# bridgedp/hunter_bipedal_control

Measured on NVIDIA H100. Metric: MPC+WBC control-step solves/sec (Hunter N=100), higher is better.
Workload: dtype f64

## Files before the change

hunter_bipedal_control_b200/csrc/hb_qp.cuh:

```cuda
#pragma once
#include "hb_common.cuh"

namespace hb {

constexpr int QP_MAX_N = 80;
constexpr int QP_MAX_EQ = 32;
constexpr int QP_MAX_IN = 96;
constexpr int QP_MAX_M = 160;

struct QpWorkspace {
  double *H, *Aeq, *K, *V, *S;
  double *kdi, *sdi;
  double *g, *x, *rd, *dx, *t1, *t2;
  double *beq, *y, *rp, *dy, *t3;
  double *f, *s, *z, *rs, *ds, *dz, *rc, *sgn, *wt;
  int *in_row, *in_c0, *in_c1, *in_pair, *ord, *eq_row;
  int ldn, ldv, lds;
  int me_cap, mi_cap;
};

__host__ __device__ constexpr int qp_ld(int n) { return n | 1; }

__host__ __device__ constexpr int tri_row(int i) { return i * (i + 1) / 2; }

__host__ __device__ constexpr size_t qp_workspace_doubles(int n, int me_cap = QP_MAX_EQ, int mi_cap = QP_MAX_IN, bool packed_h = false) {
  const int ldn = qp_ld(n), lde = me_cap | 1;
  size_t d = 0;
  d += packed_h ? (size_t)tri_row(n) : (size_t)n * ldn;
  d += (size_t)me_cap * ldn;
  d += (size_t)n * ldn;
  d += (size_t)n * lde;
  d += (size_t)me_cap * lde;
  d += n + me_cap;
  d += 6 * (size_t)n;
  d += 5 * (size_t)me_cap;
  d += 9 * (size_t)mi_cap;
  d += (5 * (size_t)mi_cap + me_cap + 1) / 2 + 1;
  return d;
}

__device__ inline void qp_carve(double* base, int n, QpWorkspace& w, int me_cap = QP_MAX_EQ, int mi_cap = QP_MAX_IN, bool packed_h = false) {
  const int ldn = qp_ld(n), lde = me_cap | 1;
  w.ldn = ldn; w.ldv = lde; w.lds = lde; w.me_cap = me_cap; w.mi_cap = mi_cap;
  double* p = base;
  w.H = p; p += packed_h ? tri_row(n) : n * ldn;
  w.Aeq = p; p += me_cap * ldn;
  w.K = p; p += n * ldn;
  w.V = p; p += n * lde;
  w.S = p; p += me_cap * lde;
  w.kdi = p; p += n;
  w.sdi = p; p += me_cap;
  w.g = p; p += n; w.x = p; p += n; w.rd = p; p += n; w.dx = p; p += n; w.t1 = p; p += n; w.t2 = p; p += n;
  w.beq = p; p += me_cap; w.y = p; p += me_cap; w.rp = p; p += me_cap; w.dy = p; p += me_cap; w.t3 = p; p += me_cap;
  w.f = p; p += mi_cap; w.s = p; p += mi_cap; w.z = p; p += mi_cap; w.rs = p; p += mi_cap;
  w.ds = p; p += mi_cap; w.dz = p; p += mi_cap; w.rc = p; p += mi_cap; w.sgn = p; p += mi_cap; w.wt = p; p += mi_cap;
  int* ip = reinterpret_cast<int*>(p);
  w.in_row = ip; ip += mi_cap; w.in_c0 = ip; ip += mi_cap; w.in_c1 = ip; ip += mi_cap; w.in_pair = ip; ip += mi_cap; w.ord = ip; ip += mi_cap; w.eq_row = ip;
}

__device__ inline bool warp_chol_inv(double* M, int n, int ld, double* invdiag, int lane, double piv_floor = 0.0) {
  bool ok = true;
  for (int j = 0; j < n; ++j) {
    for (int i = j + lane; i < n; i += 32) {
      const double* ri = M + i * ld;
      const double* rj = M + j * ld;
      double a0 = ri[j], a1 = 0.0, a2 = 0.0, a3 = 0.0;
      int k = 0;
      for (; k + 3 < j; k += 4) {
        a0 -= ri[k] * rj[k]; a1 -= ri[k + 1] * rj[k + 1]; a2 -= ri[k + 2] * rj[k + 2]; a3 -= ri[k + 3] * rj[k + 3];
      }
      for (; k < j; ++k) a0 -= ri[k] * rj[k];
      M[i * ld + j] = (a0 + a1) + (a2 + a3);
    }
    __syncwarp();
    double d = M[j * ld + j];
    if (!(d > piv_floor)) {
      if (piv_floor > 0.0 && d == d) d = piv_floor; else { ok = false; d = 1.0; }
    }
    const double r = 1.0 / sqrt(d);
    __syncwarp();
    for (int i = j + lane; i < n; i += 32) M[i * ld + j] *= r;
    if (lane == 0) invdiag[j] = r;
    __syncwarp();
  }
  for (int c0 = 0; c0 < n; c0 += 32) {
    const int c = c0 + lane;
    const bool act = c < n;
    for (int i = c0 + 1; i < n; ++i) {
      if (act && i > c) {
        const double* Li_row = M + i * ld;
        double* col = M + c * ld;
        double a0 = Li_row[c] * invdiag[c], a1 = 0.0;
        int k = c + 1;
        for (; k + 1 < i; k += 2) { a0 += Li_row[k] * col[k]; a1 += Li_row[k + 1] * col[k + 1]; }
        if (k < i) a0 += Li_row[k] * col[k];
        col[i] = -(a0 + a1) * invdiag[i];
      }
    }
  }
  __syncwarp();
  return ok;
}

template <int LD, int W, int WMAX>
__device__ __forceinline__ void chol_window_factor(double (&a)[WMAX], double* M, int& j, int jend, int n, double* invdiag, int lane,
                                                   double piv_floor, bool& ok) {
  for (; j < jend; ++j) {
    double d = __shfl_sync(HB_FULL_MASK, a[0], j);
    if (!(d > piv_floor)) { if (piv_floor > 0.0 && d == d) d = piv_floor; else { ok = false; d = 1.0; } }
    const double r = rsqrt(d);
    const double l = a[0] * r;
    if (lane < n) M[lane * LD + j] = l;
    if (lane == j) invdiag[j] = r;
    __syncwarp();
    const double* col = M + (j + 1) * LD + j;
#pragma unroll
    for (int k = 0; k < W - 1; ++k) a[k] = fma(-l, col[k * LD], a[k + 1]);
  }
}

template <int LD, int W, int WMAX>
__device__ __forceinline__ void chol_window_inverse(double (&res)[WMAX], double* M, int& j, int jend, const double* invdiag, int lane) {
  for (; j < jend; ++j) {
    const double y = res[0] * invdiag[j];
    if (lane < j) M[lane * LD + j] = y;
    const double* col = M + (j + 1) * LD + j;
#pragma unroll
    for (int k = 0; k < W - 1; ++k) res[k] = fma(-col[k * LD], y, res[k + 1]);
  }
}

template <int LD, int WMAX>
__device__ __noinline__ bool warp_chol_inv_window(double* M, int n, double* invdiag, int lane, double piv_floor) {
  static_assert(WMAX <= 32 && WMAX % 7 == 0, "one lane per row, stages of seven columns");
  bool ok = true;
  double a[WMAX];
#pragma unroll
  for (int c = 0; c < WMAX; ++c) a[c] = (lane < n && c <= lane) ? M[lane * LD + c] : 0.0;
  __syncwarp();
  int j = 0;
  if constexpr (WMAX >= 28) chol_window_factor<LD, 28, WMAX>(a, M, j, n - 21, n, invdiag, lane, piv_floor, ok);
  if constexpr (WMAX >= 21) chol_window_factor<LD, 21, WMAX>(a, M, j, n - 14, n, invdiag, lane, piv_floor, ok);
  if constexpr (WMAX >= 14) chol_window_factor<LD, 14, WMAX>(a, M, j, n - 7, n, invdiag, lane, piv_floor, ok);
  chol_window_factor<LD, 7, WMAX>(a, M, j, n, n, invdiag, lane, piv_floor, ok);
  __syncwarp();
#pragma unroll
  for (int c = 0; c < WMAX; ++c) a[c] = (c == lane) ? 1.0 : 0.0;
  j = 0;
  if constexpr (WMAX >= 28) chol_window_inverse<LD, 28, WMAX>(a, M, j, n - 21, invdiag, lane);
  if constexpr (WMAX >= 21) chol_window_inverse<LD, 21, WMAX>(a, M, j, n - 14, invdiag, lane);
  if constexpr (WMAX >= 14) chol_window_inverse<LD, 14, WMAX>(a, M, j, n - 7, invdiag, lane);
  chol_window_inverse<LD, 7, WMAX>(a, M, j, n, invdiag, lane);
  __syncwarp();
  return ok;
}

__device__ inline bool warp_chol_inv_any(double* M, int n, int ld, double* invdiag, int lane, double piv_floor) {
  if (ld == 29 && n <= 28) return warp_chol_inv_window<29, 28>(M, n, invdiag, lane, piv_floor);
  if (ld == 7 && n <= 7) return warp_chol_inv_window<7, 7>(M, n, invdiag, lane, piv_floor);
  return warp_chol_inv(M, n, ld, invdiag, lane, piv_floor);
}

__device__ inline void warp_li_mv(const double* M, int n, int ld, const double* invdiag, const double* v, double* y, int lane) {
  for (int i = lane; i < n; i += 32) {
    double a0 = invdiag[i] * v[i], a1 = 0.0;
    int k = 0;
    for (; k + 1 < i; k += 2) { a0 += M[k * ld + i] * v[k]; a1 += M[(k + 1) * ld + i] * v[k + 1]; }
    if (k < i) a0 += M[k * ld + i] * v[k];
    y[i] = a0 + a1;
  }
  __syncwarp();
}
__device__ inline void warp_lit_mv(const double* M, int n, int ld, const double* invdiag, const double* v, double* y, int lane) {
  for (int i = lane; i < n; i += 32) {
    const double* row = M + i * ld;
    double a0 = invdiag[i] * v[i], a1 = 0.0;
    int k = i + 1;
    for (; k + 1 < n; k += 2) { a0 += row[k] * v[k]; a1 += row[k + 1] * v[k + 1]; }
    if (k < n) a0 += row[k] * v[k];
    y[i] = a0 + a1;
  }
  __syncwarp();
}

struct QpResult { int status; int iters; };

template <class Bound, class Residuals, class Factor, class Newton, class Step>
__device__ __forceinline__ QpResult qp_mehrotra_warp(int mi, int max_iter, double gs, double bs, double fsum, double* s, double* z, double* ds,
                                                     double* dz, double* rc, Bound bound, Residuals residuals, Factor factor, Newton newton,
                                                     Step step) {
  const int lane = lane_id();
  fsum = warp_sum(fsum);
  const double theta = fmax(1.0, mi > 0 ? fsum / mi : 1.0);
  for (int j = lane; j < mi; j += 32) { const double sj = fmax(theta, bound(j)); s[j] = sj; z[j] = theta / sj; }
  gs = warp_max(gs); bs = warp_max(bs);
  __syncwarp();
  auto max_step = [&]() {
    double a = 1.0;
    for (int j = lane; j < mi; j += 32) {
      if (ds[j] < 0.0) a = fmin(a, -s[j] / ds[j]);
      if (dz[j] < 0.0) a = fmin(a, -z[j] / dz[j]);
    }
    return warp_min(a);
  };
  QpResult res{1, 0};
  int it = 0;
  for (; it < max_iter; ++it) {
    double rdn = 0.0, rpn = 0.0;
    const double sz = residuals(rdn, rpn);
    rdn = warp_max(rdn); rpn = warp_max(rpn);
    const double mu = mi > 0 ? warp_sum(sz) / mi : 0.0;
    if (!(rdn == rdn) || !(rpn == rpn) || !(mu == mu) || rdn > 1e300 || rpn > 1e300) { res.status = 3; break; }
    if (rdn < 1e-10 * gs && rpn < 1e-10 * bs && mu < 1e-12) { res.status = 0; break; }
    if (!factor()) { res.status = 2; break; }
    for (int j = lane; j < mi; j += 32) rc[j] = s[j] * z[j];
    __syncwarp();
    newton();
    if (mi > 0) {
      const double a_aff = max_step();
      double ma = 0.0;
      for (int j = lane; j < mi; j += 32) ma += (s[j] + a_aff * ds[j]) * (z[j] + a_aff * dz[j]);
      ma = warp_sum(ma) / mi;
      const double r = ma / mu;
      const double sigma = r * r * r;
      for (int j = lane; j < mi; j += 32) rc[j] = s[j] * z[j] + ds[j] * dz[j] - sigma * mu;
      __syncwarp();
      newton();
    }
    const double alpha = fmin(1.0, 0.995 * max_step());
    step(alpha);
    for (int j = lane; j < mi; j += 32) { s[j] += alpha * ds[j]; z[j] += alpha * dz[j]; }
    __syncwarp();
  }
  res.iters = it;
  return res;
}

template <bool PACKED_H = false>
__device__ inline QpResult qp_solve_warp(int n, int m, const double* __restrict__ H, const double* __restrict__ g,
                                         const double* __restrict__ A, const double* __restrict__ lbA,
                                         const double* __restrict__ ubA, double rho, int max_iter, double* x_out,
                                         QpWorkspace& w) {
  const int lane = lane_id();
  const int ldn = w.ldn, ldv = w.ldv, lds = w.lds;
  int me = 0, mi = 0;
  bool infeasible = false;
  for (int r0 = 0; r0 < m; r0 += 32) {
    const int r = r0 + lane;
    int c0 = n, c1 = 0;
    double lo = 0.0, hi = 0.0;
    if (r < m) {
      const double* a = A + (size_t)r * n;
      for (int c = 0; c < n; ++c) if (a[c] != 0.0) { if (c < c0) c0 = c; c1 = c + 1; }
      lo = lbA[r]; hi = ubA[r];
    }
    const bool valid = r < m;
    const bool zero_row = valid && c1 == 0;
    const bool has_lo = valid && lo > -1e19, has_hi = valid && hi < 1e19;
    if (zero_row && ((has_lo && lo > 1e-12) || (has_hi && hi < -1e-12))) infeasible = true;
    const bool is_eq = valid && !zero_row && has_lo && has_hi && lo == hi;
    const bool up = valid && !zero_row && !is_eq && has_hi;
    const bool dn = valid && !zero_row && !is_eq && has_lo;
    const unsigned beq = __ballot_sync(HB_FULL_MASK, is_eq);
    const unsigned bup = __ballot_sync(HB_FULL_MASK, up);
    const unsigned bdn = __ballot_sync(HB_FULL_MASK, dn);
    const unsigned below = (1u << lane) - 1u;
    if (is_eq) { const int e = me + __popc(beq & below); if (e < w.me_cap) { w.eq_row[e] = r; w.beq[e] = hi; } }
    const int mi2 = mi + __popc(bup);
    const int e_up = mi + __popc(bup & below), e_dn = mi2 + __popc(bdn & below);
    if (up && e_up < w.mi_cap) { w.in_row[e_up] = r; w.in_c0[e_up] = c0; w.in_c1[e_up] = c1; w.sgn[e_up] = 1.0; w.f[e_up] = hi; w.in_pair[e_up] = (dn && e_dn < w.mi_cap) ? e_dn : -1; }
    if (dn && e_dn < w.mi_cap) { w.in_row[e_dn] = r; w.in_c0[e_dn] = c0; w.in_c1[e_dn] = c1; w.sgn[e_dn] = -1.0; w.f[e_dn] = -lo; w.in_pair[e_dn] = up ? -2 : -1; }
    me += __popc(beq);
    mi = mi2 + __popc(bdn);
  }
  infeasible = __any_sync(HB_FULL_MASK, infeasible);
  QpResult res{1, 0};
  if (infeasible) res.status = 2;
  else if (me > w.me_cap || mi > w.mi_cap || n > QP_MAX_N) res.status = 4;
  if (res.status != 1) {
    for (int i = lane; i < n; i += 32) x_out[i] = 0.0;
    return res;
  }
  __syncwarp();
  int nwide = 0, nact = 0;
  for (int pass = 0; pass < 2; ++pass) {
    for (int j0 = 0; j0 < mi; j0 += 32) {
      const int j = j0 + lane;
      const bool sel = j < mi && w.in_pair[j] != -2 && ((w.in_c1[j] - w.in_c0[j] > 8) == (pass == 0));
      const unsigned msk = __ballot_sync(HB_FULL_MASK, sel);
      if (sel) w.ord[nact + __popc(msk & ((1u << lane) - 1u))] = j;
      nact += __popc(msk);
    }
    if (pass == 0) nwide = nact;
  }
  __syncwarp();
  const bool colmask = n <= 32 && nact - nwide <= 32;
  unsigned nmask = 0u;
  if (colmask && lane < n)
    for (int q = nwide; q < nact; ++q) { const int j = w.ord[q]; if (lane >= w.in_c0[j] && lane < w.in_c1[j]) nmask |= 1u << (q - nwide); }
  auto at_mul = [&](int i, double a) {
    for (int q = 0; q < nwide; ++q) { const int j = w.ord[q]; a = fma(w.wt[j], A[(size_t)w.in_row[j] * n + i], a); }
    if (colmask) {
      for (unsigned mk = nmask; mk; mk &= mk - 1u) { const int j = w.ord[nwide + __ffs(mk) - 1]; a = fma(w.wt[j], A[(size_t)w.in_row[j] * n + i], a); }
      return a;
    }
    for (int q = nwide; q < nact; ++q) {
      const int j = w.ord[q];
      if (i >= w.in_c0[j] && i < w.in_c1[j]) a = fma(w.wt[j], A[(size_t)w.in_row[j] * n + i], a);
    }
    return a;
  };
  if (H != nullptr) for (int idx = lane; idx < n * n; idx += 32) { const int i = idx / n, c = idx - i * n; w.H[i * ldn + c] = H[idx]; }
  for (int e = 0; e < me; ++e) {
    const double* a = A + (size_t)w.eq_row[e] * n;
    for (int c = lane; c < n; c += 32) w.Aeq[e * ldn + c] = a[c];
  }
  double gs = 1.0, bs = 1.0;
  for (int i = lane; i < n; i += 32) { const double gi = g[i]; w.g[i] = gi; w.x[i] = 0.0; gs = fmax(gs, 1.0 + fabs(gi)); }
  for (int e = lane; e < me; e += 32) { w.y[e] = 0.0; bs = fmax(bs, 1.0 + fabs(w.beq[e])); }
  double fsum = 0.0;
  for (int j = lane; j < mi; j += 32) { fsum += fabs(w.f[j]); bs = fmax(bs, 1.0 + fabs(w.f[j])); }
  auto residuals = [&](double& rdn, double& rpn) {
    for (int j = lane; j < mi; j += 32) {
      const int pr = w.in_pair[j];
      double cj = w.sgn[j] * w.z[j];
      if (pr >= 0) cj += w.sgn[pr] * w.z[pr];
      w.wt[j] = cj;
    }
    __syncwarp();
    for (int i = lane; i < n; i += 32) {
      double a = w.g[i] + rho * w.x[i];
      if (PACKED_H) {
        const double* hr = w.H + tri_row(i);
        for (int c = 0; c <= i; ++c) a += hr[c] * w.x[c];
        for (int c = i + 1; c < n; ++c) a += w.H[tri_row(c) + i] * w.x[c];
      } else {
        const double* hr = w.H + i * ldn;
        for (int c = 0; c < n; ++c) a += hr[c] * w.x[c];
      }
      for (int e = 0; e < me; ++e) a += w.Aeq[e * ldn + i] * w.y[e];
      w.rd[i] = at_mul(i, a);
    }
    for (int e = lane; e < me; e += 32) {
      double a = -w.beq[e];
      for (int c = 0; c < n; ++c) a += w.Aeq[e * ldn + c] * w.x[c];
      w.rp[e] = a;
    }
    double sz = 0.0;
    for (int j = lane; j < mi; j += 32) {
      const double* a = A + (size_t)w.in_row[j] * n;
      double d = 0.0;
      for (int c = w.in_c0[j]; c < w.in_c1[j]; ++c) d += a[c] * w.x[c];
      w.rs[j] = w.sgn[j] * d + w.s[j] - w.f[j];
      sz += w.s[j] * w.z[j];
    }
    __syncwarp();
    for (int i = lane; i < n; i += 32) rdn = fmax(rdn, fabs(w.rd[i]));
    for (int e = lane; e < me; e += 32) rpn = fmax(rpn, fabs(w.rp[e]));
    for (int j = lane; j < mi; j += 32) rpn = fmax(rpn, fabs(w.rs[j]));
    return sz;
  };
  auto factor = [&]() {
    if (PACKED_H) {
      for (int idx = lane; idx < n * ldn; idx += 32) { const int i = idx / ldn, c = idx - i * ldn; if (c <= i) w.K[idx] = w.H[tri_row(i) + c] + ((i == c) ? rho : 0.0); }
    } else {
      for (int idx = lane; idx < n * ldn; idx += 32) { const int i = idx / ldn, c = idx - i * ldn; w.K[idx] = w.H[idx] + ((i == c) ? rho : 0.0); }
    }
    __syncwarp();
    for (int j = lane; j < mi; j += 32) {
      const int pr = w.in_pair[j];
      double wj = w.z[j] / w.s[j];
      if (pr >= 0) wj += w.z[pr] / w.s[pr];
      w.wt[j] = wj;
    }
    __syncwarp();
    {
      constexpr int WCH = 10;
      for (int cb = 0; cb < n; cb += 32) {
        const int c = cb + lane;
        const bool act = c < n;
        for (int q0 = 0; q0 < nwide; q0 += WCH) {
          double t[WCH]; int roff[WCH];
#pragma unroll
          for (int q = 0; q < WCH; ++q) {
            const bool on = q0 + q < nwide;
            const int j = on ? w.ord[q0 + q] : 0;
            roff[q] = on ? w.in_row[j] * n : 0;
            t[q] = (on && act) ? w.wt[j] * A[(size_t)roff[q] + c] : 0.0;
          }
          for (int i = cb; i < n; ++i) {
            double acc = 0.0;
#pragma unroll
            for (int q = 0; q < WCH; ++q) acc = fma(t[q], A[(size_t)roff[q] + i], acc);
            if (act && i >= c) w.K[i * ldn + c] += acc;
          }
        }
      }
    }
    __syncwarp();
    if (colmask) {
      for (unsigned mk = nmask; mk; mk &= mk - 1u) {
        const int j = w.ord[nwide + __ffs(mk) - 1];
        const int c1 = w.in_c1[j];
        const double wj = w.wt[j];
        const double* a = A + (size_t)w.in_row[j] * n;
        const double ac = a[lane];
        for (int i = lane; i < c1; ++i) w.K[i * ldn + lane] += (wj * a[i]) * ac;
      }
      __syncwarp();
    } else
    for (int q = nwide; q < nact; ++q) {
      const int j = w.ord[q];
      const int c0 = w.in_c0[j], c1 = w.in_c1[j];
      const double wj = w.wt[j];
      const double* a = A + (size_t)w.in_row[j] * n;
      for (int i = c0; i < c1; ++i) {
        const double ai = wj * a[i];
        for (int c = c0 + lane; c <= i; c += 32) w.K[i * ldn + c] += ai * a[c];
      }
      __syncwarp();
    }
    bool ok = warp_chol_inv_any(w.K, n, ldn, w.kdi, lane, 1e-10);
    if (me > 0) {
      for (int idx = lane; idx < n * me; idx += 32) {
        const int i = idx / me, e = idx - i * me;
        const double* ar = w.Aeq + e * ldn;
        double a0 = w.kdi[i] * ar[i], a1 = 0.0;
        int k = 0;
        for (; k + 1 < i; k += 2) { a0 += w.K[k * ldn + i] * ar[k]; a1 += w.K[(k + 1) * ldn + i] * ar[k + 1]; }
        if (k < i) a0 += w.K[k * ldn + i] * ar[k];
        w.V[i * ldv + e] = a0 + a1;
      }
      __syncwarp();
      for (int idx = lane; idx < me * me; idx += 32) {
        const int a = idx / me, b = idx - a * me;
        if (b <= a) {
          double s0 = 0.0, s1 = 0.0;
          int i = 0;
          for (; i + 1 < n; i += 2) { s0 += w.V[i * ldv + a] * w.V[i * ldv + b]; s1 += w.V[(i + 1) * ldv + a] * w.V[(i + 1) * ldv + b]; }
          if (i < n) s0 += w.V[i * ldv + a] * w.V[i * ldv + b];
          w.S[a * lds + b] = s0 + s1;
        }
      }
      __syncwarp();
      ok = warp_chol_inv_any(w.S, me, lds, w.sdi, lane, 1e-14) && ok;
    }
    return ok;
  };
  auto newton = [&]() {
    for (int j = lane; j < mi; j += 32) {
      const int pr = w.in_pair[j];
      double cj = w.sgn[j] * ((w.rc[j] - w.z[j] * w.rs[j]) / w.s[j]);
      if (pr >= 0) cj += w.sgn[pr] * ((w.rc[pr] - w.z[pr] * w.rs[pr]) / w.s[pr]);
      w.wt[j] = cj;
    }
    __syncwarp();
    for (int i = lane; i < n; i += 32) w.t2[i] = at_mul(i, -w.rd[i]);
    __syncwarp();
    warp_li_mv(w.K, n, ldn, w.kdi, w.t2, w.t1, lane);
    if (me > 0) {
      for (int e = lane; e < me; e += 32) {
        double a = w.rp[e];
        for (int i = 0; i < n; ++i) a += w.V[i * ldv + e] * w.t1[i];
        w.t3[e] = a;
      }
      __syncwarp();
      warp_li_mv(w.S, me, lds, w.sdi, w.t3, w.dy, lane);
      for (int e = lane; e < me; e += 32) w.t3[e] = w.dy[e];
      __syncwarp();
      warp_lit_mv(w.S, me, lds, w.sdi, w.t3, w.dy, lane);
      for (int i = lane; i < n; i += 32) {
        double a = w.t1[i];
        for (int e = 0; e < me; ++e) a -= w.V[i * ldv + e] * w.dy[e];
        w.t2[i] = a;
      }
      __syncwarp();
    } else {
      for (int i = lane; i < n; i += 32) w.t2[i] = w.t1[i];
      __syncwarp();
    }
    warp_lit_mv(w.K, n, ldn, w.kdi, w.t2, w.dx, lane);
    for (int j = lane; j < mi; j += 32) {
      const double* a = A + (size_t)w.in_row[j] * n;
      double d = 0.0;
      for (int c = w.in_c0[j]; c < w.in_c1[j]; ++c) d += a[c] * w.dx[c];
      const double dsj = -w.rs[j] - w.sgn[j] * d;
      w.ds[j] = dsj;
      w.dz[j] = -(w.rc[j] + w.z[j] * dsj) / w.s[j];
    }
    __syncwarp();
  };
  auto step = [&](double alpha) {
    for (int i = lane; i < n; i += 32) w.x[i] += alpha * w.dx[i];
    for (int e = lane; e < me; e += 32) w.y[e] += alpha * w.dy[e];
  };
  res = qp_mehrotra_warp(mi, max_iter, gs, bs, fsum, w.s, w.z, w.ds, w.dz, w.rc, [&](int j) { return w.f[j]; }, residuals, factor, newton, step);
  for (int i = lane; i < n; i += 32) x_out[i] = w.x[i];
  return res;
}

}

namespace {
using namespace hb;
__global__ void qp_batch_kernel(int B, int n, int m, const double* H, const double* g, const double* A, const double* lbA, const double* ubA,
                                size_t strideH, size_t strideA, size_t strideB, const int32_t* m_per, double rho, int max_iter, double* x,
                                int32_t* status, int32_t* iters) {
  extern __shared__ __align__(16) unsigned char smem_raw[];
  const int warp = threadIdx.x >> 5, wpb = blockDim.x >> 5;
  const int inst = blockIdx.x * wpb + warp;
  if (inst >= B) return;
  double* base = reinterpret_cast<double*>(smem_raw) + (size_t)warp * qp_workspace_doubles(n);
  QpWorkspace w;
  qp_carve(base, n, w);
  const int mi = m_per ? m_per[inst] : m;
  QpResult r = qp_solve_warp(n, mi, H + inst * strideH, g + (size_t)inst * n, A + inst * strideA, lbA + inst * strideB, ubA + inst * strideB,
                             rho, max_iter, x + (size_t)inst * n, w);
  if (lane_id() == 0) { if (status) status[inst] = r.status; if (iters) iters[inst] = r.iters; }
}
}
```

hunter_bipedal_control_b200/csrc/hb_wbc.cuh:

```cuda
#pragma once
#include "hb_common.cuh"
#include "hb_planner.h"
#include "hb_qp.cuh"
#include "hb_rbd.cuh"
#include "../../include/hunter_b200.h"

namespace hb {

constexpr int WBC_ROWS = 60;
constexpr double QP_INFTY = 1e20;

struct WbcShared {
  double J[12 * 16];
  double Ad[6 * 16];
  double M[16 * 16];
  double nle[16];
  double q[16], v[16], qd[16], vd[16];
  double pos_m[12], vel_m[12], dJv[12], pos_d[12], vel_d[12];
  double Adv[6], com_d[3];
  double At[18 * 16];
  double bt[18];
  double misc[32];
  double frame[36];
};

struct WbcRows {
  int nc, nsw;
  int eq;
  int md0;
  int nt;
  int ma2;
  int m;
};
__device__ inline WbcRows wbc_rows(int mode, bool stance_mode) {
  int nc = 0;
  for (int c = 0; c < 4; ++c) nc += contact_flag(mode, c);
  const int nsw = 4 - nc, eq = 16 + 3 * nsw, md0 = 2 * NJ + 5 * nc;
  return {nc, nsw, eq, md0, stance_mode ? 6 : 3 * nsw + 6, 12 + 3 * nsw, eq + md0 + 3 * nsw};
}
constexpr int WBC_MA0 = 28;

__device__ inline void rotation_error_world(const double* Rref, const double* Rmeas, double* err) {
  double E[9];
  for (int i = 0; i < 3; ++i)
    for (int j = 0; j < 3; ++j) E[3 * i + j] = Rref[3 * i] * Rmeas[3 * j] + Rref[3 * i + 1] * Rmeas[3 * j + 1] + Rref[3 * i + 2] * Rmeas[3 * j + 2];
  const double sk[3] = {E[7] - E[5], E[2] - E[6], E[3] - E[1]};
  double c = 0.5 * (E[0] + E[4] + E[8] - 1.0);
  c = fmin(1.0, fmax(-1.0, c));
  const double ang = acos(c);
  const double sn = sqrt(sk[0] * sk[0] + sk[1] * sk[1] + sk[2] * sk[2]);
  double f = 0.5;
  if (ang > 1e-8 && sn > 1e-12) f = ang / sn;
  for (int i = 0; i < 3; ++i) err[i] = f * sk[i];
}

__device__ inline void wbc_contact_frames(const hb_terrain& m, WbcShared& sh) {
  const int c = lane_id();
  if (c >= 4) return;
  double* f = sh.frame + 9 * c;
  if (!hbplan::map_frame(m, sh.pos_m[3 * c], sh.pos_m[3 * c + 1], f)) f[2] = 0.0;
}

__device__ __forceinline__ const double* wbc_frames(const InstanceView<hb_terrain>& maps, int inst, const WbcShared& sh) {
  return maps.of(inst) ? sh.frame : nullptr;
}

__device__ inline int wbc_terms_warp(const double* __restrict__ x_des, const double* __restrict__ u_des, const double* __restrict__ rbd,
                                     int mode, const bool& stance_mode, const hb_wbc_settings& ws, const InstanceView<hb_terrain>& maps, int inst,
                                     WbcShared& sh) {
  const int lane = lane_id();
  const Model& md = c_model;
  if (lane == 0) {
    rbd_to_qv(rbd, sh.q, sh.v);
    for (int i = 0; i < NQ; ++i) sh.qd[i] = x_des[6 + i];
  }
  __syncwarp();
  {
    double q[NQ], e[NQ];
    const bool meas = lane < 16;
    const int k = lane & 15;
    for (int i = 0; i < NQ; ++i) { q[i] = meas ? sh.q[i] : sh.qd[i]; e[i] = (i == k) ? 1.0 : 0.0; }
    KinOut<double> o;
    kin_pass<double>(q, e, o);
    if (meas) { for (int r = 0; r < 12; ++r) sh.J[r * 16 + k] = o.cvel[r]; }
    else { for (int r = 0; r < 6; ++r) sh.Ad[r * 16 + k] = o.h[r]; }
  }
  __syncwarp();
  if (lane == 0) {
    double Ab[36], rhs[6], vb[6];
    for (int r = 0; r < 6; ++r) {
      for (int c = 0; c < 6; ++c) Ab[6 * r + c] = sh.Ad[r * 16 + c];
      double s = md.total_mass * x_des[r];
      for (int j = 0; j < NJ; ++j) s -= sh.Ad[r * 16 + 6 + j] * u_des[12 + j];
      rhs[r] = s;
    }
    solve6_cmm(Ab, rhs, vb);
    for (int i = 0; i < 6; ++i) sh.vd[i] = vb[i];
    for (int j = 0; j < NJ; ++j) sh.vd[6 + j] = u_des[12 + j];
  }
  __syncwarp();
  if (lane < 2) {
    D1 q[NQ], v[NQ];
    for (int i = 0; i < NQ; ++i) {
      const double qi = lane == 0 ? sh.q[i] : sh.qd[i], vi = lane == 0 ? sh.v[i] : sh.vd[i];
      q[i] = D1(qi, vi); v[i] = D1(vi, 0.0);
    }
    KinOut<D1> o;
    kin_pass<D1>(q, v, o);
    if (lane == 0) { for (int r = 0; r < 12; ++r) { sh.pos_m[r] = o.cpos[r].v; sh.vel_m[r] = o.cvel[r].v; sh.dJv[r] = o.cvel[r].d; } }
    else {
      for (int r = 0; r < 12; ++r) { sh.pos_d[r] = o.cpos[r].v; sh.vel_d[r] = o.cvel[r].v; }
      for (int r = 0; r < 6; ++r) sh.Adv[r] = o.h[r].d;
      for (int r = 0; r < 3; ++r) sh.com_d[r] = o.com[r].v;
    }
  }
  if (lane < 17) {
    double q[NQ], v[NQ], a[NQ], tau[NQ];
    for (int i = 0; i < NQ; ++i) { q[i] = sh.q[i]; v[i] = lane == 16 ? sh.v[i] : 0.0; a[i] = (i == lane) ? 1.0 : 0.0; }
    rnea_pass(q, v, a, lane == 16, tau, nullptr);
    if (lane < 16) { for (int r = 0; r < NQ; ++r) sh.M[r * 16 + lane] = tau[r]; }
    else { for (int r = 0; r < NQ; ++r) sh.nle[r] = tau[r]; }
  }
  __syncwarp();
  if (const hb_terrain* m = maps.of(inst)) wbc_contact_frames(*m, sh);
  for (int idx = lane; idx < 256; idx += 32) {
    const int i = idx >> 4, j = idx & 15;
    if (j < i) { const double a = 0.5 * (sh.M[i * 16 + j] + sh.M[j * 16 + i]); sh.M[i * 16 + j] = a; }
  }
  __syncwarp();
  for (int idx = lane; idx < 256; idx += 32) { const int i = idx >> 4, j = idx & 15; if (j > i) sh.M[i * 16 + j] = sh.M[j * 16 + i]; }
  __syncwarp();
  if (lane == 0) {
    bool fl[4];
    for (int c = 0; c < 4; ++c) fl[c] = contact_flag(mode, c);
    for (int i = 0; i < 18 * 16; ++i) sh.At[i] = 0.0;
    if (stance_mode) {
      for (int i = 0; i < 6; ++i) { sh.At[i * 16 + i] = 1.0; sh.bt[i] = 0.0; }
    } else {
      double hd[6] = {0, 0, 0, 0, 0, 0};
      for (int c = 0; c < 4; ++c) {
        const double* F = u_des + 3 * c;
        const double r0 = sh.pos_d[3 * c] - sh.com_d[0], r1 = sh.pos_d[3 * c + 1] - sh.com_d[1], r2 = sh.pos_d[3 * c + 2] - sh.com_d[2];
        hd[0] += F[0]; hd[1] += F[1]; hd[2] += F[2];
        hd[3] += r1 * F[2] - r2 * F[1]; hd[4] += r2 * F[0] - r0 * F[2]; hd[5] += r0 * F[1] - r1 * F[0];
      }
      hd[2] -= md.total_mass * HB_GRAVITY;
      double Ab[36], rhs[6], qbdd[6];
      for (int r = 0; r < 6; ++r) { for (int c = 0; c < 6; ++c) Ab[6 * r + c] = sh.Ad[r * 16 + c]; rhs[r] = hd[r] - sh.Adv[r]; }
      solve6_cmm(Ab, rhs, qbdd);
      double Rd[9], axd[9], Rm[9], axm[9];
      base_frame<double>(sh.qd, Rd, axd);
      base_frame<double>(sh.q, Rm, axm);
      double baseVelW[3], baseAccW[3], wm[3], dJw_v[3];
      {
        const double* vd = sh.vd;
        double w1[3], w2[3], t1[3], t2[3];
        for (int i = 0; i < 3; ++i) { w1[i] = axd[i] * vd[3]; w2[i] = w1[i] + axd[3 + i] * vd[4]; }
        cross(w1, &axd[3], t1); cross(w2, &axd[6], t2);
        for (int i = 0; i < 3; ++i) {
          baseVelW[i] = w2[i] + axd[6 + i] * vd[5];
          baseAccW[i] = axd[i] * qbdd[3] + axd[3 + i] * qbdd[4] + axd[6 + i] * qbdd[5] + t1[i] * vd[4] + t2[i] * vd[5];
        }
      }
      {
        const double* vm = sh.v;
        double w1[3], w2[3], t1[3], t2[3];
        for (int i = 0; i < 3; ++i) { w1[i] = axm[i] * vm[3]; w2[i] = w1[i] + axm[3 + i] * vm[4]; }
        cross(w1, &axm[3], t1); cross(w2, &axm[6], t2);
        for (int i = 0; i < 3; ++i) { wm[i] = w2[i] + axm[6 + i] * vm[5]; dJw_v[i] = t1[i] * vm[4] + t2[i] * vm[5]; }
      }
      int r = 0;
      for (int c = 0; c < 4; ++c) if (!fl[c]) for (int a = 0; a < 3; ++a) {
        const double acc = ws.swing_kp * (sh.pos_d[3 * c + a] - sh.pos_m[3 * c + a]) + ws.swing_kd * (sh.vel_d[3 * c + a] - sh.vel_m[3 * c + a]);
        for (int j = 0; j < NQ; ++j) sh.At[r * 16 + j] = sh.J[(3 * c + a) * 16 + j];
        sh.bt[r] = acc - sh.dJv[3 * c + a];
        ++r;
      }
      for (int a = 0; a < 2; ++a) { sh.At[r * 16 + a] = 1.0; sh.bt[r] = qbdd[a]; ++r; }
      sh.At[r * 16 + 2] = 1.0;
      sh.bt[r] = qbdd[2] + ws.base_height_kp * (sh.qd[2] - sh.q[2]) + ws.base_height_kd * (sh.vd[2] - sh.v[2]);
      ++r;
      double err[3];
      rotation_error_world(Rd, Rm, err);
      for (int a = 0; a < 3; ++a) {
        for (int i = 0; i < 3; ++i) sh.At[r * 16 + 3 + i] = axm[3 * i + a];
        sh.bt[r] = baseAccW[a] + ws.base_angular_kp * err[a] + ws.base_angular_kd * (baseVelW[a] - wm[a]) - dJw_v[a];
        ++r;
      }
    }
  }
  __syncwarp();
  return wbc_rows(mode, stance_mode).nt;
}

__device__ inline void wbc_weight_rows(WbcShared& sh, const WbcRows& n, bool stance_mode, const hb_wbc_settings& ws) {
  const int lane = lane_id(), nsr = stance_mode ? 0 : 3 * n.nsw;
  for (int idx = lane; idx < n.nt * 16; idx += 32) sh.At[idx] *= (idx >> 4) < nsr ? ws.weight_swing_leg : ws.weight_base_accel;
  for (int r = lane; r < n.nt; r += 32) sh.bt[r] *= r < nsr ? ws.weight_swing_leg : ws.weight_base_accel;
  __syncwarp();
}

__device__ inline const hb_wbc_settings& wbc_select_settings(const hb_wbc_settings& ws, InstanceView<hb_controller_setting> cs, int inst,
                                                             hb_wbc_settings& dst) {
  if (lane_id() == 0) {
    const hb_controller_setting* c = cs.of(inst);
    if (c) dst = c->wbc;
    else dst = ws;
  }
  __syncwarp();
  return dst;
}

__device__ inline int wbc_nth_contact(int mode, bool stance, int k) {
  int c = 0;
  for (; c < 3; ++c) if (contact_flag(mode, c) == stance && k-- == 0) break;
  return c;
}

__device__ inline void wbc_task0_eq(const WbcShared& sh, int mode, const WbcRows& n, int rows, double* A, int lda, double* b) {
  const int lane = lane_id(), nsw = n.nsw;
  for (int idx = lane; idx < rows * NWBC; idx += 32) {
    const int i = idx / NWBC, j = idx - i * NWBC;
    double a = 0.0;
    if (i < 16) {
      if (j < NQ) a = sh.M[i * 16 + j];
      else if (j < NQ + 12) a = -sh.J[(j - NQ) * 16 + i];
      else a = (i >= 6 && j - NQ - 12 == i - 6) ? -1.0 : 0.0;
    } else if (i < 16 + 3 * nsw) {
      const int k = i - 16, c = wbc_nth_contact(mode, false, k / 3);
      a = (j == NQ + 3 * c + k % 3) ? 1.0 : 0.0;
    } else {
      const int k = i - 16 - 3 * nsw, c = wbc_nth_contact(mode, true, k / 3);
      a = j < NQ ? sh.J[(3 * c + k % 3) * 16 + j] : 0.0;
    }
    A[i * lda + j] = a;
  }
  for (int i = lane; i < rows; i += 32) {
    double v = 0.0;
    if (i < 16) v = -sh.nle[i];
    else if (i >= 16 + 3 * nsw) { const int k = i - 16 - 3 * nsw; v = -sh.dJv[3 * wbc_nth_contact(mode, true, k / 3) + k % 3]; }
    b[i] = v;
  }
}

__device__ inline double wbc_task0_ineq(const hb_wbc_settings& ws, int mode, int q, int& col0, int& len, double* coef, const double* frames) {
  if (q < 2 * NJ) {
    const int j = q % NJ;
    col0 = NQ + 12 + j; len = 1; coef[0] = q < NJ ? 1.0 : -1.0; coef[1] = 0.0; coef[2] = 0.0;
    return ws.torque_limits[j % 5];
  }
  const int fr = q - 2 * NJ, k = fr % 5;
  const double mu = ws.friction_coefficient;
  const int c = wbc_nth_contact(mode, true, fr / 5);
  col0 = NQ + 3 * c; len = 3;
  const double* f = frames ? frames + 9 * c : nullptr;
  if (f && f[2] != 0.0) {
    const double* t = f + (k < 3 ? 3 : 6);
    for (int a = 0; a < 3; ++a) coef[a] = k == 0 ? -f[a] : (k & 1 ? t[a] : -t[a]) - hbplan::mul_rn(mu, f[a]);
    return 0.0;
  }
  coef[0] = k == 1 ? 1.0 : (k == 2 ? -1.0 : 0.0);
  coef[1] = k == 3 ? 1.0 : (k == 4 ? -1.0 : 0.0);
  coef[2] = k == 0 ? -1.0 : -mu;
  return 0.0;
}

__device__ inline int wbc_task12_rows(int lvl, const double* At, const double* bt, const WbcRows& n, const double* u_des, double* A, int lda, double* b) {
  const int lane = lane_id(), nswr = 3 * n.nsw;
  const int ma = lvl == 1 ? 6 : n.ma2;
  for (int idx = lane; idx < ma * NWBC; idx += 32) {
    const int i = idx / NWBC, j = idx - i * NWBC;
    double a = 0.0;
    if (lvl == 1) { if (j < NQ) a = At[(nswr + i) * 16 + j]; }
    else if (i < 12) a = (j == NQ + i) ? 0.1 : 0.0;
    else if (j < NQ) a = At[(i - 12) * 16 + j];
    A[i * lda + j] = a;
  }
  for (int i = lane; i < ma; i += 32) b[i] = lvl == 1 ? bt[nswr + i] : (i < 12 ? 0.1 * u_des[i] : bt[i - 12]);
  return ma;
}

__device__ inline int wbc_reduced_build(const WbcShared& sh, const WbcRows& n, int mode, bool stance_mode, double rho, const hb_wbc_settings& ws,
                                        const double* frames, const double* __restrict__ u_des, double* Hw, double* gz, double* Az, double* lbz,
                                        double* ubz, int* stcol , int& m_out) {
  const int lane = lane_id();
  if (lane == 0) for (int j = 0, k = 0; j < 12; ++j) if (contact_flag(mode, j / 3)) stcol[k++] = j;
  const int nz = NQ + 3 * n.nc, m = 6 + NJ + 5 * n.nc, nw = n.nt;
  __syncwarp();
  for (int idx = lane; idx < m * nz; idx += 32) {
    const int r = idx / nz, c = idx - r * nz;
    double v = 0.0;
    if (r < 6 + NJ) v = (c < NQ) ? sh.M[r * 16 + c] : -sh.J[stcol[c - NQ] * 16 + r];
    else {
      const int fr = r - 6 - NJ, ci = fr / 5;
      const int cc = c - NQ - 3 * ci;
      if (cc >= 0 && cc < 3) { int c0, len; double coef[3]; wbc_task0_ineq(ws, mode, 2 * NJ + fr, c0, len, coef, frames); v = coef[cc]; }
    }
    Az[idx] = v;
  }
  for (int r = lane; r < m; r += 32) {
    int c0, len; double coef[3];
    if (r < 6) { lbz[r] = -sh.nle[r]; ubz[r] = -sh.nle[r]; }
    else if (r < 6 + NJ) { const int j = r - 6; const double lim = wbc_task0_ineq(ws, mode, j, c0, len, coef, nullptr); lbz[r] = -lim - sh.nle[6 + j]; ubz[r] = lim - sh.nle[6 + j]; }
    else { lbz[r] = -QP_INFTY; ubz[r] = wbc_task0_ineq(ws, mode, NJ + r - 6, c0, len, coef, frames); }
  }
  __syncwarp();
  const double* Tm = Az + 6 * nz;
  const double wf2 = stance_mode ? 0.0 : ws.weight_contact_force * ws.weight_contact_force;
  for (int idx = lane; idx < nz * nz; idx += 32) {
    const int i = idx / nz, j = idx - i * nz;
    if (j > i) continue;
    double s = (i == j) ? rho : 0.0;
    if (i == j && i >= NQ) s += wf2;
    if (i < NQ && j < NQ) for (int r = 0; r < nw; ++r) s += sh.At[r * 16 + i] * sh.At[r * 16 + j];
    double t = 0.0;
    for (int r = 0; r < NJ; ++r) t += Tm[r * nz + i] * Tm[r * nz + j];
    Hw[tri_row(i) + j] = s + rho * t;
  }
  for (int i = lane; i < nz; i += 32) {
    double s = 0.0;
    if (i < NQ) for (int r = 0; r < nw; ++r) s -= sh.At[r * 16 + i] * sh.bt[r];
    else s = -wf2 * u_des[stcol[i - NQ]];
    double t = 0.0;
    for (int r = 0; r < NJ; ++r) t += Tm[r * nz + i] * sh.nle[6 + r];
    gz[i] = s + rho * t;
  }
  __syncwarp();
  m_out = m;
  return nz;
}

}

namespace {
using namespace hb;
constexpr int QP_STRIDE_H = NWBC * NWBC, QP_STRIDE_A = WBC_ROWS * NWBC;

__global__ void wbc_assemble_kernel(int B, hb_wbc_settings ws, const __grid_constant__ InstanceView<hb_terrain> maps, const double* x_des,
                                    const double* u_des, const double* rbd, const int32_t* mode, const uint8_t* stance_mode, double* H, double* g,
                                    double* A, double* lbA, double* ubA, int32_t* m_out) {
  extern __shared__ __align__(16) unsigned char smem_raw[];
  const int warp = threadIdx.x >> 5, wpb = blockDim.x >> 5;
  const int inst = blockIdx.x * wpb + warp;
  if (inst >= B) return;
  WbcShared& sh = reinterpret_cast<WbcShared*>(smem_raw)[warp];
  const int md = mode[inst];
  const bool stance = stance_mode ? stance_mode[inst] != 0 : false;
  const double* ud = u_des + (size_t)inst * NU;
  wbc_terms_warp(x_des + (size_t)inst * NX, ud, rbd + (size_t)inst * 32, md, stance, ws, maps, inst, sh);
  const WbcRows n = wbc_rows(md, stance);
  wbc_weight_rows(sh, n, stance, ws);
  const int lane = lane_id();
  H += (size_t)inst * QP_STRIDE_H; g += (size_t)inst * NWBC; A += (size_t)inst * QP_STRIDE_A; lbA += (size_t)inst * WBC_ROWS; ubA += (size_t)inst * WBC_ROWS;
  const double wf2 = stance ? 0.0 : ws.weight_contact_force * ws.weight_contact_force;
  for (int idx = lane; idx < NWBC * NWBC; idx += 32) {
    const int i = idx / NWBC, j = idx - i * NWBC;
    double s = 0.0;
    if (i < NQ && j < NQ) for (int r = 0; r < n.nt; ++r) s += sh.At[r * 16 + i] * sh.At[r * 16 + j];
    if (i == j && i >= NQ && i < NQ + 12) s += wf2;
    H[idx] = s;
  }
  for (int i = lane; i < NWBC; i += 32) {
    double s = 0.0;
    if (i < NQ) for (int r = 0; r < n.nt; ++r) s += sh.At[r * 16 + i] * sh.bt[r];
    else if (i < NQ + 12) s = wf2 * ud[i - NQ];
    g[i] = -s;
  }
  for (int idx = lane; idx < n.m * NWBC; idx += 32) A[idx] = 0.0;
  __syncwarp();
  wbc_task0_eq(sh, md, n, n.eq, A, NWBC, lbA);
  for (int q = lane; q < n.md0; q += 32) {
    int c0, len; double coef[3];
    const int r = n.eq + q;
    ubA[r] = wbc_task0_ineq(ws, md, q, c0, len, coef, wbc_frames(maps, inst, sh));
    lbA[r] = -QP_INFTY;
    for (int k = 0; k < len; ++k) A[r * NWBC + c0 + k] = coef[k];
  }
  for (int r = n.eq + n.md0 + lane; r < n.m; r += 32) { lbA[r] = -QP_INFTY; ubA[r] = 0.0; }
  __syncwarp();
  for (int i = lane; i < n.eq; i += 32) ubA[i] = lbA[i];
  if (lane == 0) m_out[inst] = n.m;
}

constexpr int WZ_N = 28, WZ_ME = 6, WZ_MI = 40, WZ_ROWS = 36;
__host__ __device__ constexpr size_t wbc_fused_doubles() { return qp_workspace_doubles(WZ_N, WZ_ME, WZ_MI, true) + WZ_ROWS * WZ_N + 2 * WZ_ROWS + 3 * WZ_N + 16 + 8; }
static_assert(8 * (wbc_fused_doubles() * sizeof(double) + 1024) <= 228 * 1024, "wbc_fused_kernel must fit 8 blocks per SM");

struct WbcStaged { WbcShared sh; hb_wbc_settings ws; bool stance; };

__global__ void __launch_bounds__(32, 8) wbc_fused_kernel(int B, hb_wbc_settings ws_ctx, InstanceView<hb_controller_setting> cs,
                                 const __grid_constant__ InstanceView<hb_terrain> maps, const double* x_des, const double* u_des, const double* rbd,
                                 const int32_t* mode, const uint8_t* stance_mode, double rho, int max_iter, double* sol, int32_t* status, int32_t* iters) {
  extern __shared__ __align__(16) unsigned char smem_raw[];
  const int warp = threadIdx.x >> 5, wpb = blockDim.x >> 5, lane = threadIdx.x & 31;
  const int inst = blockIdx.x * wpb + warp;
  if (inst >= B) return;
  double* base = reinterpret_cast<double*>(smem_raw) + (size_t)warp * wbc_fused_doubles();
  QpWorkspace w;
  qp_carve(base, WZ_N, w, WZ_ME, WZ_MI, true);
  double* p = base + qp_workspace_doubles(WZ_N, WZ_ME, WZ_MI, true);
  double* Az = p; p += WZ_ROWS * WZ_N;
  double* lbz = p; p += WZ_ROWS;
  double* ubz = p; p += WZ_ROWS;
  double* gz = p; p += WZ_N;
  double* xz = p; p += WZ_N;
  double* nlej = p; p += WZ_N;
  int* stcol = reinterpret_cast<int*>(p);
  static_assert(sizeof(WbcStaged) <= sizeof(double) * (WZ_N * 29 + WZ_N * 7 + WZ_ME * 7 + WZ_N + WZ_ME + 6 * WZ_N + 5 * WZ_ME + 8 * WZ_MI), "assembly scratch must fit in the aliased area");
  WbcStaged& stg = *reinterpret_cast<WbcStaged*>(w.K);
  WbcShared& sh = stg.sh;
  if (lane == 0) stg.stance = stance_mode ? stance_mode[inst] != 0 : false;
  const hb_wbc_settings& ws = wbc_select_settings(ws_ctx, cs, inst, stg.ws);
  const int md = mode[inst];
  wbc_terms_warp(x_des + (size_t)inst * NX, u_des + (size_t)inst * NU, rbd + (size_t)inst * 32, md, stg.stance, ws, maps, inst, sh);
  const bool stance = stg.stance;
  const WbcRows n = wbc_rows(md, stance);
  wbc_weight_rows(sh, n, stance, ws);
  int m = 0;
  const int nz = wbc_reduced_build(sh, n, md, stance, rho, ws, wbc_frames(maps, inst, sh), u_des + (size_t)inst * NU, w.H, gz, Az, lbz, ubz, stcol, m);
  if (lane < NJ) nlej[lane] = sh.nle[6 + lane];
  __syncwarp();
  QpResult r = qp_solve_warp<true>(nz, m, nullptr, gz, Az, lbz, ubz, 0.0, max_iter, xz, w);
  __syncwarp();
  double* out = sol + (size_t)inst * NWBC;
  if (lane < NQ) out[lane] = xz[lane];
  if (lane < 12) {
    double f = 0.0;
    for (int c = 0; c < nz - NQ; ++c) if (stcol[c] == lane) f = xz[NQ + c];
    out[NQ + lane] = f;
  }
  if (lane < NJ) {
    double t = nlej[lane];
    for (int c = 0; c < nz; ++c) t += Az[(6 + lane) * nz + c] * xz[c];
    out[NQ + 12 + lane] = t;
  }
  if (lane == 0) { if (status) status[inst] = r.status; if (iters) iters[inst] = r.iters; }
}

__global__ void torque_kernel(int B, const double* sol, double* torque) {
  const int idx = blockIdx.x * blockDim.x + threadIdx.x;
  if (idx < B * NJ) { const int i = idx / NJ, j = idx - i * NJ; torque[idx] = sol[(size_t)i * NWBC + 28 + j]; }
}

__global__ void wbc_fallback_kernel(int B, int have_prev, const int32_t* status, double* sol, double* prev, double* torque) {
  const int idx = blockIdx.x * blockDim.x + threadIdx.x;
  if (idx >= B * NWBC) return;
  const int i = idx / NWBC, j = idx - i * NWBC;
  if (status[i] != 0 && have_prev) {
    const double v = prev[idx];
    sol[idx] = v;
    if (torque && j >= 28) torque[(size_t)i * NJ + j - 28] = v;
  } else {
    prev[idx] = sol[idx];
  }
}
}
```

Before: 189,600.

## Outline WBC QP solve into noinline call and tune packed-H QP loops

```diff
diff --git a/hunter_bipedal_control_b200/csrc/hb_qp.cuh b/hunter_bipedal_control_b200/csrc/hb_qp.cuh
--- a/hunter_bipedal_control_b200/csrc/hb_qp.cuh
+++ b/hunter_bipedal_control_b200/csrc/hb_qp.cuh
@@ -299,7 +299,12 @@
   if (colmask && lane < n)
     for (int q = nwide; q < nact; ++q) { const int j = w.ord[q]; if (lane >= w.in_c0[j] && lane < w.in_c1[j]) nmask |= 1u << (q - nwide); }
   auto at_mul = [&](int i, double a) {
-    for (int q = 0; q < nwide; ++q) { const int j = w.ord[q]; a = fma(w.wt[j], A[(size_t)w.in_row[j] * n + i], a); }
+    if constexpr (PACKED_H) {
+#pragma unroll 5
+      for (int q = 0; q < nwide; ++q) { const int j = w.ord[q]; a = fma(w.wt[j], A[(size_t)w.in_row[j] * n + i], a); }
+    } else {
+      for (int q = 0; q < nwide; ++q) { const int j = w.ord[q]; a = fma(w.wt[j], A[(size_t)w.in_row[j] * n + i], a); }
+    }
     if (colmask) {
       for (unsigned mk = nmask; mk; mk &= mk - 1u) { const int j = w.ord[nwide + __ffs(mk) - 1]; a = fma(w.wt[j], A[(size_t)w.in_row[j] * n + i], a); }
       return a;
@@ -331,9 +336,8 @@
     for (int i = lane; i < n; i += 32) {
       double a = w.g[i] + rho * w.x[i];
       if (PACKED_H) {
-        const double* hr = w.H + tri_row(i);
-        for (int c = 0; c <= i; ++c) a += hr[c] * w.x[c];
-        for (int c = i + 1; c < n; ++c) a += w.H[tri_row(c) + i] * w.x[c];
+        const int ri = tri_row(i);
+        for (int c = 0; c < n; ++c) a += w.H[c <= i ? ri + c : tri_row(c) + i] * w.x[c];
       } else {
         const double* hr = w.H + i * ldn;
         for (int c = 0; c < n; ++c) a += hr[c] * w.x[c];
@@ -362,7 +366,7 @@
   };
   auto factor = [&]() {
     if (PACKED_H) {
-      for (int idx = lane; idx < n * ldn; idx += 32) { const int i = idx / ldn, c = idx - i * ldn; if (c <= i) w.K[idx] = w.H[tri_row(i) + c] + ((i == c) ? rho : 0.0); }
+      for (int i = 0; i < n; ++i) for (int c = lane; c <= i; c += 32) w.K[i * ldn + c] = w.H[tri_row(i) + c] + ((i == c) ? rho : 0.0);
     } else {
       for (int idx = lane; idx < n * ldn; idx += 32) { const int i = idx / ldn, c = idx - i * ldn; w.K[idx] = w.H[idx] + ((i == c) ? rho : 0.0); }
     }
@@ -388,11 +392,17 @@
             roff[q] = on ? w.in_row[j] * n : 0;
             t[q] = (on && act) ? w.wt[j] * A[(size_t)roff[q] + c] : 0.0;
           }
-          for (int i = cb; i < n; ++i) {
+          auto wide_row = [&](int i) {
             double acc = 0.0;
 #pragma unroll
             for (int q = 0; q < WCH; ++q) acc = fma(t[q], A[(size_t)roff[q] + i], acc);
             if (act && i >= c) w.K[i * ldn + c] += acc;
+          };
+          if constexpr (PACKED_H) {
+#pragma unroll 2
+            for (int i = cb; i < n; ++i) wide_row(i);
+          } else {
+            for (int i = cb; i < n; ++i) wide_row(i);
           }
         }
       }
diff --git a/hunter_bipedal_control_b200/csrc/hb_wbc.cuh b/hunter_bipedal_control_b200/csrc/hb_wbc.cuh
--- a/hunter_bipedal_control_b200/csrc/hb_wbc.cuh
+++ b/hunter_bipedal_control_b200/csrc/hb_wbc.cuh
@@ -129,11 +129,11 @@
   }
   __syncwarp();
   for (int idx = lane; idx < 256; idx += 32) { const int i = idx >> 4, j = idx & 15; if (j > i) sh.M[i * 16 + j] = sh.M[j * 16 + i]; }
+  for (int idx = lane; idx < 18 * 16; idx += 32) sh.At[idx] = 0.0;
   __syncwarp();
   if (lane == 0) {
     bool fl[4];
     for (int c = 0; c < 4; ++c) fl[c] = contact_flag(mode, c);
-    for (int i = 0; i < 18 * 16; ++i) sh.At[i] = 0.0;
     if (stance_mode) {
       for (int i = 0; i < 6; ++i) { sh.At[i * 16 + i] = 1.0; sh.bt[i] = 0.0; }
     } else {
@@ -388,24 +388,38 @@
 
 struct WbcStaged { WbcShared sh; hb_wbc_settings ws; bool stance; };
 
+struct WbcFusedArea { QpWorkspace w; double *Az, *lbz, *ubz, *gz, *xz, *nlej; int* stcol; };
+__device__ __forceinline__ WbcFusedArea wbc_fused_area() {
+  extern __shared__ __align__(16) unsigned char smem_raw[];
+  WbcFusedArea a;
+  double* base = reinterpret_cast<double*>(smem_raw) + (size_t)(threadIdx.x >> 5) * wbc_fused_doubles();
+  qp_carve(base, WZ_N, a.w, WZ_ME, WZ_MI, true);
+  double* p = base + qp_workspace_doubles(WZ_N, WZ_ME, WZ_MI, true);
+  a.Az = p; p += WZ_ROWS * WZ_N;
+  a.lbz = p; p += WZ_ROWS;
+  a.ubz = p; p += WZ_ROWS;
+  a.gz = p; p += WZ_N;
+  a.xz = p; p += WZ_N;
+  a.nlej = p; p += WZ_N;
+  a.stcol = reinterpret_cast<int*>(p);
+  return a;
+}
+
+__device__ __noinline__ QpResult wbc_fused_qp(int nz, int m, int max_iter) {
+  WbcFusedArea a = wbc_fused_area();
+  return qp_solve_warp<true>(nz, m, nullptr, a.gz, a.Az, a.lbz, a.ubz, 0.0, max_iter, a.xz, a.w);
+}
+
 __global__ void __launch_bounds__(32, 8) wbc_fused_kernel(int B, hb_wbc_settings ws_ctx, InstanceView<hb_controller_setting> cs,
                                  const __grid_constant__ InstanceView<hb_terrain> maps, const double* x_des, const double* u_des, const double* rbd,
                                  const int32_t* mode, const uint8_t* stance_mode, double rho, int max_iter, double* sol, int32_t* status, int32_t* iters) {
-  extern __shared__ __align__(16) unsigned char smem_raw[];
   const int warp = threadIdx.x >> 5, wpb = blockDim.x >> 5, lane = threadIdx.x & 31;
   const int inst = blockIdx.x * wpb + warp;
   if (inst >= B) return;
-  double* base = reinterpret_cast<double*>(smem_raw) + (size_t)warp * wbc_fused_doubles();
-  QpWorkspace w;
-  qp_carve(base, WZ_N, w, WZ_ME, WZ_MI, true);
-  double* p = base + qp_workspace_doubles(WZ_N, WZ_ME, WZ_MI, true);
-  double* Az = p; p += WZ_ROWS * WZ_N;
-  double* lbz = p; p += WZ_ROWS;
-  double* ubz = p; p += WZ_ROWS;
-  double* gz = p; p += WZ_N;
-  double* xz = p; p += WZ_N;
-  double* nlej = p; p += WZ_N;
-  int* stcol = reinterpret_cast<int*>(p);
+  const WbcFusedArea area = wbc_fused_area();
+  const QpWorkspace& w = area.w;
+  double *Az = area.Az, *lbz = area.lbz, *ubz = area.ubz, *gz = area.gz, *xz = area.xz, *nlej = area.nlej;
+  int* stcol = area.stcol;
   static_assert(sizeof(WbcStaged) <= sizeof(double) * (WZ_N * 29 + WZ_N * 7 + WZ_ME * 7 + WZ_N + WZ_ME + 6 * WZ_N + 5 * WZ_ME + 8 * WZ_MI), "assembly scratch must fit in the aliased area");
   WbcStaged& stg = *reinterpret_cast<WbcStaged*>(w.K);
   WbcShared& sh = stg.sh;
@@ -420,7 +434,7 @@
   const int nz = wbc_reduced_build(sh, n, md, stance, rho, ws, wbc_frames(maps, inst, sh), u_des + (size_t)inst * NU, w.H, gz, Az, lbz, ubz, stcol, m);
   if (lane < NJ) nlej[lane] = sh.nle[6 + lane];
   __syncwarp();
-  QpResult r = qp_solve_warp<true>(nz, m, nullptr, gz, Az, lbz, ubz, 0.0, max_iter, xz, w);
+  QpResult r = wbc_fused_qp(nz, m, max_iter);
   __syncwarp();
   double* out = sol + (size_t)inst * NWBC;
   if (lane < NQ) out[lane] = xz[lane];
```

New measurement: 191,700 (median of 6 runs). +1.1%, better.
